# cxjyxxme/deep-online-video-stabilization

Measured on AMD Instinct MI355X. Metric: stabilized frames/sec (720p, before_ch=31), higher is better.
Workload: dtype f32 (bf16x3 split MFMA, f32 accumulate); 1 GPU; BASELINE.json configs[1]: v2_93 net, 1280x720, 1 stream(s)/GPU, batch=1 per stream, 13-ch stack from a 32-deep ring (lags 1,2,4,8,16,32; --before-ch 31 ignored as in the reference), ResNet-v2-50 regressor + 4x4 multi-grid warp + feedback; one independent stream set per GPU (replicas only); height=720, width=1280, streams_per_gpu=1, refine=1, operand_mode=4, launches_per_frame=64, hip_graph=True

## Files before the change

deep-online-video-stabilization_amd/csrc/conv.h:

```cpp
#pragma once
#include "common.h"

struct ConvArgs {
    const float* x;
    const float* w;
    float* y;
    const float* bias;
    const float* in_scale;
    const float* in_shift;
    const float* residual;
    const float* out_scale;
    const float* out_shift;
    const float* out_floor;
    float* partial;
    int N, H, W, Cin, Ho, Wo, Cout, KH, KW, stride, pad;
    int up;
    int res_H, res_W, res_stride;
    int relu_out;
    int x_ld, res_ld;
    int M, K;
    int splitk, steps_per_split;
    int cin_real;
    unsigned div_hw_mul, div_hw_shift, div_w_mul, div_w_shift;
    int rowrun;
    int in_scale_expected;
    int xcd_swizzle;
};

size_t conv_plan(ConvArgs& a);
struct Prof;
int conv_launch(const ConvArgs& a, hipStream_t st, Prof* prof = nullptr, int bf16_operands = 0, const float* w_img = nullptr,
                bool lowk_ring = false);

enum ConvFamily {
    CONV_IGEMM,
    CONV_RING,
    CONV_RING_KG,
    CONV_RING_PRO,
    CONV_PACKED,
    CONV_PACKED_KG2,
    CONV_ASTAT,
    CONV_PATCH
};
struct ConvRoute {
    int family;
    int tile, bk, nbuf;
    int mode;
    int operand;
    int kg, pro;
    int reduce;
    int prof_kind;
    int astat_bm;
    int patch_cfg;
};
ConvRoute conv_route(const ConvArgs& a, int operand_mode, bool has_image, bool bound, bool lowk_ring = false );
const char* conv_prof_kind_name(int kind);
size_t conv_weight_image_floats(int Cout, int K);
int launch_weight_split_image(const float* w, int Cout, int K, float* img, hipStream_t st);
struct WeightImageTable { long w_off[64], img_off[64], tprefix[65]; int Cout[64], K[64]; int n; };
void weight_image_table_add(WeightImageTable& t, long w_off, long img_off, int Cout, int K);
int launch_weight_split_images(const float* w_base, float* img_base, const WeightImageTable& t, hipStream_t st);
int conv_reduce_launches(const ConvArgs& a, int operand_mode = 0);

struct ConvPair { int m_tower, x_tower_floats ; long dx, dy, dres, dscale; };
bool conv_pair_supported(const ConvArgs& a);
int conv_launch_pair(const ConvArgs& a, const ConvPair& pr, hipStream_t st, Prof* prof = nullptr,
                     const float* w_img = nullptr );

bool conv_b2b_supported(const ConvArgs& c2, const ConvArgs& c3);
int conv_b2b_launch(const ConvArgs& c2, const ConvArgs& c3, hipStream_t st, Prof* prof = nullptr);

static inline void sn_fastdiv_make(unsigned d, unsigned& mul, unsigned& shift) {
    unsigned l = 0;
    while ((1ull << l) < d) ++l;
    mul = (unsigned)((((1ull << l) - d) << 32) / d + 1);
    shift = l;
}
#ifdef __HIPCC__
__device__ __forceinline__ int sn_fastdiv(int n, unsigned mul, unsigned shift) {
    return (int)((__umulhi(mul, (unsigned)n) + (unsigned)n) >> shift);
}
#endif
```

deep-online-video-stabilization_amd/csrc/conv.hip:

```cpp
#include "conv.h"
#include "prof.h"
#include <climits>
#include <cstdio>
#include <cstdlib>
#include <algorithm>
#include <string>
#include <vector>

#include "conv_kernel.h"
#include "conv_ring_kernel.h"
#include "conv_astat_kernel.h"
#include "conv_patch_kernel.h"
#include "conv_b2b_kernel.h"

template <int PAIR>
__device__ __forceinline__ void conv_splitk_reduce_body(const ConvArgs& p, const ConvPair& pr) {
    const size_t q = (size_t)blockIdx.x * 256 + threadIdx.x;
    const int c4n = p.Cout / 4;
    if (q >= (size_t)p.M * c4n) return;
    const int m = (int)(q / c4n);
    const int n = (int)(q - (size_t)m * c4n) * 4;
    const bool t1 = PAIR && m >= pr.m_tower;
    const size_t slab = (size_t)p.M * p.Cout;
    const float* src = p.partial + (size_t)m * p.Cout + n;
    float4 s = *reinterpret_cast<const float4*>(src);
    for (int z = 1; z < p.splitk; ++z) {
        const float4 t = *reinterpret_cast<const float4*>(src + z * slab);
        s.x += t.x; s.y += t.y; s.z += t.z; s.w += t.w;
    }
    if (p.bias != nullptr) {
        const float4 b = *reinterpret_cast<const float4*>(p.bias + n);
        s.x += b.x; s.y += b.y; s.z += b.z; s.w += b.w;
    }
    if (p.residual != nullptr) {
        size_t ri;
        if (p.res_stride == 1 && p.res_H == p.Ho && p.res_W == p.Wo) {
            ri = (size_t)m * p.res_ld + n;
        } else {
            const int img = sn_fastdiv(m, p.div_hw_mul, p.div_hw_shift);
            const int rr = m - img * (p.Ho * p.Wo);
            const int oy = sn_fastdiv(rr, p.div_w_mul, p.div_w_shift), ox = rr - oy * p.Wo;
            ri = (((size_t)img * p.res_H + oy * p.res_stride) * p.res_W + ox * p.res_stride) * p.res_ld + n;
        }
        const float4 t = *reinterpret_cast<const float4*>(p.residual + (t1 ? pr.dres : 0) + ri);
        s.x += t.x; s.y += t.y; s.z += t.z; s.w += t.w;
    }
    if (p.out_scale != nullptr) {
        const float4 a = *reinterpret_cast<const float4*>(p.out_scale + n), b = *reinterpret_cast<const float4*>(p.out_shift + n);
        s.x = __builtin_fmaf(s.x, a.x, b.x); s.y = __builtin_fmaf(s.y, a.y, b.y);
        s.z = __builtin_fmaf(s.z, a.z, b.z); s.w = __builtin_fmaf(s.w, a.w, b.w);
    }
    if (p.out_scale != nullptr && p.out_floor != nullptr) {
        const float4 f = *reinterpret_cast<const float4*>(p.out_floor + n);
        s.x = fmaxf(s.x, f.x); s.y = fmaxf(s.y, f.y); s.z = fmaxf(s.z, f.z); s.w = fmaxf(s.w, f.w);
    } else if (p.relu_out) {
        s.x = fmaxf(s.x, 0.f); s.y = fmaxf(s.y, 0.f); s.z = fmaxf(s.z, 0.f); s.w = fmaxf(s.w, 0.f);
    }
    *reinterpret_cast<float4*>(p.y + (t1 ? pr.dy : 0) + (size_t)m * p.Cout + n) = s;
}
__global__ __launch_bounds__(256) void conv_splitk_reduce_kernel(const ConvArgs p) {
    conv_splitk_reduce_body<0>(p, ConvPair{});
}
__global__ __launch_bounds__(256) void conv_splitk_reduce_pair_kernel(const ConvArgs p, const ConvPair pr) {
    conv_splitk_reduce_body<1>(p, pr);
}

enum TileId { T128x128 = 0, T128x64 = 1, T64x64 = 2 };

static void tile_dims(int t, int& bm, int& bn) {
    bm = (t == T64x64) ? 64 : 128;
    bn = (t == T128x128) ? 128 : 64;
}

static int env_int(const char* name, int dflt) {
    const char* v = getenv(name);
    return v ? atoi(v) : dflt;
}

struct ConvSwitches {
    int tile = env_int("STABNET_CONV_TILE", -1), splitk = env_int("STABNET_CONV_SPLITK", -1);
    int bk16 = env_int("STABNET_CONV_BK16", 0);
    int nbuf = env_int("STABNET_CONV_NBUF", 0);
    int tuning_table = env_int("STABNET_CONV_TUNING_TABLE", 1);
    int split_below = env_int("STABNET_CONV_SPLIT_BELOW", 400), split_target = env_int("STABNET_CONV_SPLIT_TARGET", 448);
    int xcd = env_int("STABNET_CONV_XCD", 1);
    int ring = env_int("STABNET_CONV_RING", 1), ring_wgs_per_cu = env_int("STABNET_CONV_RING_WGS_PER_CU", 3);
    int lowk_igemm = env_int("STABNET_CONV_LOWK_IGEMM", 1);
    int ring_pro = env_int("STABNET_CONV_RING_PRO", 1);
    int kgroups = env_int("STABNET_CONV_KGROUPS", 1), kgroups_pro = env_int("STABNET_CONV_KGROUPS_PRO", 1);
    int packed_kg2 = env_int("STABNET_CONV_PACKED_KG2", 1), packed_kg3 = env_int("STABNET_CONV_PACKED_KG3", 1);
    int packed_pro = env_int("STABNET_CONV_PACKED_PRO", 1);
    int packed_wgs_per_cu = env_int("STABNET_CONV_PACKED_WGS_PER_CU", 2);
    int astat = env_int("STABNET_CONV_ASTAT", 1), astat_min_m = env_int("STABNET_CONV_ASTAT_MIN_M", 0);
    int astat_min_cout = env_int("STABNET_CONV_ASTAT_MIN_COUT", 256);
    int patch = env_int("STABNET_CONV_PATCH", 1), patch_min_m = env_int("STABNET_CONV_PATCH_MIN_M", 0);
    int patch_cfg = env_int("STABNET_CONV_PATCH_CFG", 0);
    int b2b = env_int("STABNET_CONV_B2B", 1), b2b_wgs_per_cu = env_int("STABNET_CONV_B2B_WGS_PER_CU", 2);
};
static const ConvSwitches& sw() {
    static const ConvSwitches s;
    return s;
}

static int g_force_tile = -2, g_force_split = -1;
static int force_tile() { return g_force_tile == -2 ? sw().tile : g_force_tile; }
static int force_split() { return g_force_tile == -2 ? sw().splitk : g_force_split; }

static int conv_bk(const ConvArgs& a) { return (a.rowrun || (a.Cin % 32 == 0 && !sw().bk16)) ? 32 : 16; }
static int conv_total_steps(const ConvArgs& a) {
    if (a.rowrun) return a.KH * cdiv(a.KW * a.Cin, 32);
    return a.KH * a.KW * (a.Cin / conv_bk(a));
}

struct TuneEntry { int M, Cout, K, KH, ring, splitk; };
#include "conv_tuning_table.h"
#include "conv_tuning_table_packed.h"
static int g_tuning_profile = 0;
static std::vector<TuneEntry> g_tuning_runtime;

static int tuning_lookup(int M, int Cout, int K, int KH, int ring) {
    for (const TuneEntry& e : g_tuning_runtime)
        if (e.M == M && e.Cout == Cout && e.K == K && e.KH == KH && e.ring == ring) return e.splitk;
    if (sw().tuning_table && g_tuning_profile == 1)
        for (const TuneEntry& e : g_tuning_packed)
            if (e.M == M && e.Cout == Cout && e.K == K && e.KH == KH && e.ring == ring) return e.splitk;
    if (sw().tuning_table)
        for (const TuneEntry& e : g_tuning_builtin)
            if (e.M == M && e.Cout == Cout && e.K == K && e.KH == KH && e.ring == ring) return e.splitk;
    return 0;
}

static int pick_tile(const ConvArgs& a, int& splitk) {
    if (force_tile() >= 0) {
        const int steps0 = conv_total_steps(a);
        splitk = force_split() > 0 ? std::min(force_split(), steps0) : 1;
        return force_tile();
    }
    const int total_steps = conv_total_steps(a);
    const long blocks = (long)cdiv(a.M, 64) * cdiv(a.Cout, 64);
    const bool ring_path = a.rowrun || (a.in_scale_expected == 0 && a.up == 1 && a.Cin % 32 == 0);
    int s = tuning_lookup(a.M, a.Cout, a.K, a.KH, ring_path ? 1 : 0);
    const int thr = sw().split_below, target = sw().split_target;
    if (s > 0) {
        s = std::min(s, std::max(1, total_steps / 2));
    } else if (blocks < thr && a.Cout % 4 == 0) {
        s = (int)((target + blocks / 2) / blocks);
        s = std::min(s, std::max(1, total_steps / 8));
        s = std::min(s, 32);
    } else {
        s = 1;
    }
    splitk = std::max(1, s);
    return T64x64;
}

size_t conv_plan(ConvArgs& a) {
    a.xcd_swizzle = sw().xcd;
    a.M = a.N * a.Ho * a.Wo;
    a.K = a.rowrun ? a.KH * 32 * cdiv(a.KW * a.Cin, 32) : a.KH * a.KW * a.Cin;
    if (a.x_ld == 0) a.x_ld = a.Cin;
    if (a.res_ld == 0) a.res_ld = a.Cout;
    sn_fastdiv_make((unsigned)(a.Ho * a.Wo), a.div_hw_mul, a.div_hw_shift);
    sn_fastdiv_make((unsigned)a.Wo, a.div_w_mul, a.div_w_shift);
    int splitk = 1;
    (void)pick_tile(a, splitk);
    const int total_steps = conv_total_steps(a);
    a.steps_per_split = cdiv(total_steps, splitk);
    a.splitk = cdiv(total_steps, a.steps_per_split);
    return a.splitk > 1 ? (size_t)a.splitk * a.M * a.Cout * sizeof(float) : 0;
}

static void igemm_variant(const ConvArgs& a, int bm, int bn, int bk, int mode, int operand, int& nbuf_out, int& bf16_out) {
    const int nbuf = sw().nbuf;
    bf16_out = (bm == 64 && bn == 64 && bk == 32) ? operand : 0;
    const bool one_stage = nbuf == 1 || (nbuf == 0 && mode == 0 && bm == 64 && bn == 64 && a.M >= 32768);
    nbuf_out = (bf16_out != 1 && one_stage) ? 1 : 2;
}

static bool ring_eligible(const ConvArgs& a, int tile, bool has_prologue, bool lowk_ring = false) {
    if (a.rowrun) return true;
    if (!lowk_ring && sw().lowk_igemm && a.KH == 1 && a.KW == 1 && a.Cin == 64 && a.x_ld == a.Cin && a.out_floor == nullptr) return false;
    return sw().ring && tile == T64x64 && !has_prologue && a.up == 1 && a.Cin % 32 == 0 && !sw().bk16;
}

static bool ring_pro_vectors_ok(const ConvArgs& a) {
    if (a.in_scale == nullptr || a.in_shift == nullptr) return true;
    const long d = (long)(a.in_shift - a.in_scale);
    return d >= 0 && d < (1L << 30);
}
static bool ring_pro_geometry(const ConvArgs& a, int operand, bool has_prologue) {
    return sw().ring_pro && sw().ring && operand != 1 && !sw().bk16 && has_prologue && a.KH == 1 && a.KW == 1 && a.stride == 1 && a.pad == 0 &&
           a.up == 1 && a.Cin % 32 == 0 && !a.rowrun && a.x_ld == a.Cin;
}
static bool ring_pro_eligible(const ConvArgs& a, int operand) {
    return ring_pro_geometry(a, operand, a.in_scale != nullptr) && a.out_scale == nullptr && a.out_floor == nullptr && ring_pro_vectors_ok(a);
}

static int conv_kgroups(const ConvArgs& a, int operand, bool ring, bool has_prologue) {
    if (!sw().kgroups || a.splitk < 2 || operand == 1) return 1;
    if (a.steps_per_split * a.splitk != conv_total_steps(a)) return 1;
    if (ring && a.splitk == 3 && !a.rowrun) return 3;
    if (sw().kgroups_pro && !ring && a.splitk == 2 && ring_pro_geometry(a, operand, has_prologue) && ring_pro_vectors_ok(a)) return 2;
    return 1;
}

struct PatchForm { int ph, pw, wr, ns; };
static const PatchForm g_patch_forms[] = {{8, 8, 1, 3}, {8, 8, 2, 3}};
constexpr int SN_PATCH_FORMS = 2;
constexpr size_t SN_PATCH_LDS_MAX = 160 * 1024;
static int patch_cfg(const ConvArgs& a) {
    auto fits = [&](int cfg) { return sn_patch_lds_bytes(g_patch_forms[cfg - 1].ph, g_patch_forms[cfg - 1].pw, a.Cin) <= SN_PATCH_LDS_MAX; };
    const int forced = sw().patch_cfg;
    if (forced >= 1 && forced <= SN_PATCH_FORMS) return fits(forced) ? forced : 0;
    const int cfg = a.Cout <= 64 ? 1 : 2;
    return fits(cfg) ? cfg : 0;
}

static int route_prof_kind(const ConvRoute& r) {
    switch (r.family) {
        case CONV_IGEMM:
            return PK_KERNEL_CONV_BASE + r.mode * 6 + r.tile * 2 + (r.bk == 32 ? 1 : 0) + (r.nbuf == 1 ? 18 : 0) + 36 * r.operand;
        case CONV_PACKED: return PK_KERNEL_CONV_PACKED + (r.pro ? 3 : r.mode);
        case CONV_PACKED_KG2: return PK_KERNEL_CONV_PACKED + (r.pro ? 6 : 4 + r.mode);
        case CONV_ASTAT: return PK_KERNEL_CONV_ASTAT;
        case CONV_PATCH: return PK_KERNEL_CONV_PATCH + r.patch_cfg - 1;
        default: break;
    }
    const int split = r.operand >= 2 ? PK_KERNEL_CONV_SPLIT + 8 * (r.operand - 2) : 0;
    if (r.family == CONV_RING) return split ? split + r.mode : PK_KERNEL_CONV_RING + r.mode + (r.operand ? 3 : 0);
    if (r.family == CONV_RING_PRO) return split ? split + 5 : PK_KERNEL_CONV_KG + 2;
    if (r.kg == 2) return split ? split + 6 : PK_KERNEL_CONV_KG + 3;
    return split ? split + 3 + r.mode : PK_KERNEL_CONV_KG + r.mode;
}

ConvRoute conv_route(const ConvArgs& a, int operand_mode, bool has_image, bool bound, bool lowk_ring) {
    const ConvSwitches& s = sw();
    const bool image = operand_mode == 4 && has_image;
    const int op = operand_mode == 4 ? 0 : operand_mode;
    int splitk_unused = 1;
    const int t = pick_tile(a, splitk_unused);
    const bool t64 = t == T64x64, bk32 = conv_bk(a) == 32;
    const bool has_pro = bound ? a.in_scale != nullptr : a.in_scale_expected != 0;
    const bool ring = ring_eligible(a, t, has_pro, lowk_ring && image);
    const bool slabs = !bound || a.splitk == 1 || a.partial != nullptr;
    int kg = t64 ? conv_kgroups(a, op, ring, has_pro) : 1;
    if (image && s.packed_kg3 && ring && kg == 3 && a.K % 32 == 0 && slabs) kg = 1;
    const bool pro = kg == 1 && !ring && t64 && bk32 && (bound ? ring_pro_eligible(a, op) : ring_pro_geometry(a, op, has_pro));
    const bool packed_pro = image && s.packed_pro && !ring && t64 && bk32 && ring_pro_geometry(a, op, has_pro) &&
                            (!bound || a.out_floor == nullptr)  && ring_pro_vectors_ok(a) && slabs;
    if (packed_pro) kg = 1;
    const bool packed = (image && ring && kg == 1 && a.K % 32 == 0) || packed_pro;
    const bool packed_kg2 = packed && s.packed_kg2 && a.splitk == 2 && !a.rowrun && a.steps_per_split * 2 == conv_total_steps(a);
    if (packed_kg2) kg = 2;
    const int astat_min_m = s.astat_min_m > 0 ? s.astat_min_m : ((long)a.Cout * a.K >= 128 * 1024 ? 2048 : 8192);
    const bool astat = packed && !packed_pro && !packed_kg2 && kg == 1 && a.splitk == 1 && s.astat && !lowk_ring && !a.rowrun &&
                       a.KH == 1 && a.KW == 1 && a.stride == 1 && a.pad == 0 && a.up == 1 && a.K <= 256 && a.Cout >= s.astat_min_cout &&
                       a.M >= astat_min_m;
    const int patch_form = patch_cfg(a);
    const bool patch = packed && !packed_pro && ((kg == 1 && a.splitk == 1) || packed_kg2) && s.patch && !lowk_ring && !a.rowrun &&
                       a.KH == 3 && a.KW == 3 && a.stride == 1 && a.pad == 1 && a.up == 1 && a.Cin % 32 == 0 && patch_form != 0 &&
                       a.M >= (s.patch_min_m > 0 ? s.patch_min_m : 12288);

    ConvRoute r{};
    r.tile = t;
    r.bk = bk32 ? 32 : 16;
    r.mode = (a.up > 1 || a.rowrun) ? 2 : (a.pad == 0 ? 0 : 1);
    r.operand = op;
    r.kg = kg;
    r.reduce = (a.splitk > 1 && kg == 1) ? 1 : 0;
    if (astat) {
        r.family = CONV_ASTAT;
        r.operand = 4;
        r.astat_bm = 32;
    } else if (patch) {
        r.family = CONV_PATCH;
        r.operand = 4;
        r.patch_cfg = patch_form;
    } else if (packed) {
        r.family = packed_kg2 ? CONV_PACKED_KG2 : CONV_PACKED;
        r.operand = 4;
        r.pro = packed_pro ? 1 : 0;
    } else if (pro) {
        r.family = CONV_RING_PRO;
        r.pro = 1;
    } else if (kg > 1) {
        r.family = CONV_RING_KG;
        r.pro = kg == 2 ? 1 : 0;
    } else if (ring) {
        r.family = CONV_RING;
    } else {
        int bm, bn;
        tile_dims(t, bm, bn);
        r.family = CONV_IGEMM;
        igemm_variant(a, bm, bn, r.bk, r.mode, op, r.nbuf, r.operand);
    }
    r.prof_kind = route_prof_kind(r);
    return r;
}

int conv_reduce_launches(const ConvArgs& a, int operand_mode) {
    return a.splitk < 2 ? 0 : conv_route(a, operand_mode, operand_mode == 4, false).reduce;
}

const char* conv_prof_kind_name(int kind) {
    static const std::vector<std::string> names = [] {
        std::vector<std::string> v(PK_KERNEL_CONV_BASE + 144);
        char buf[96];
        auto ring = [&](int family, int mode, int operand, int kg, int pro) {
            ConvRoute r{};
            r.family = family; r.mode = mode; r.operand = operand; r.kg = kg; r.pro = pro;
            snprintf(buf, sizeof(buf), "conv_ring_f32_kernel<%d, %d, %d, %d>", mode, operand, kg, pro);
            v[route_prof_kind(r)] = buf;
        };
        for (int operand = 0; operand < 4; ++operand) {
            for (int mode = 0; mode < 3; ++mode) ring(CONV_RING, mode, operand, 1, 0);
            if (operand == 1) continue;
            ring(CONV_RING_KG, 0, operand, 3, 0); ring(CONV_RING_KG, 1, operand, 3, 0);
            ring(CONV_RING_PRO, 0, operand, 1, 1); ring(CONV_RING_KG, 0, operand, 2, 1);
        }
        for (int mode = 0; mode < 3; ++mode) ring(CONV_PACKED, mode, 4, 1, 0);
        ring(CONV_PACKED, 0, 4, 1, 1);
        ring(CONV_PACKED_KG2, 0, 4, 2, 0); ring(CONV_PACKED_KG2, 1, 4, 2, 0); ring(CONV_PACKED_KG2, 0, 4, 2, 1);
        {
            ConvRoute r{};
            r.family = CONV_ASTAT; r.astat_bm = 32;
            snprintf(buf, sizeof(buf), "conv_astat_f32_kernel<%d>", r.astat_bm);
            v[route_prof_kind(r)] = buf;
        }
        for (int cfg = 1; cfg <= SN_PATCH_FORMS; ++cfg) {
            ConvRoute r{};
            r.family = CONV_PATCH; r.patch_cfg = cfg;
            const PatchForm& f = g_patch_forms[cfg - 1];
            snprintf(buf, sizeof(buf), "conv_patch_f32_kernel<%d, %d, %d, %d>", f.ph, f.pw, f.wr, f.ns);
            v[route_prof_kind(r)] = buf;
        }
        for (int i = 0; i < 144; ++i) {
            ConvRoute r{};
            r.family = CONV_IGEMM;
            r.operand = i / 36; r.nbuf = 2 - i / 18 % 2; r.mode = i / 6 % 3; r.tile = i / 2 % 3; r.bk = (i & 1) ? 32 : 16;
            int bm, bn;
            tile_dims(r.tile, bm, bn);
            snprintf(buf, sizeof(buf), "conv_igemm_f32_kernel<%d, %d, %d, %d, %d, %d, %d, %d>", bm, bn, r.bk, bm / 2, bn / 2, r.mode, r.nbuf, r.operand);
            v[route_prof_kind(r)] = buf;
        }
        for (int i = 0; i < 4; ++i) {
            snprintf(buf, sizeof(buf), "conv_igemm_f32_pair_kernel<64, 64, %d, 32, 32, %d>", (i & 1) ? 32 : 16, i / 2);
            v[PK_KERNEL_CONV_PAIR + i] = buf;
        }
        v[PK_KERNEL_CONV_B2B] = "conv_b2b_f32_kernel<2>";
        v[PK_KERNEL_CONV_B2B + 1] = "conv_b2b_f32_kernel<4>";
        return v;
    }();
    return (kind >= 0 && kind < (int)names.size() && !names[kind].empty()) ? names[kind].c_str() : nullptr;
}

template <int BM, int BN, int BK, int WM, int WN, int MODE, int NBUF, int BF16 = 0>
static int launch_one_nb(const ConvArgs& a, hipStream_t st) {
    constexpr size_t lds_op = NBUF * (size_t)(BM + BN) * (BK + 4) * sizeof(float);
    constexpr size_t lds_epi = 4 * (size_t)SN_EPI_WAVE_BYTES;
    constexpr size_t lds = lds_op > lds_epi ? lds_op : lds_epi;
    static bool configured = false;
    auto kern = conv_igemm_f32_kernel<BM, BN, BK, WM, WN, MODE, NBUF, BF16>;
    if (!configured) {
        if (lds > 64 * 1024) {
            hipError_t e = hipFuncSetAttribute(reinterpret_cast<const void*>(kern),
                                               hipFuncAttributeMaxDynamicSharedMemorySize, (int)lds);
            if (e != hipSuccess) {
                stabnet_set_error("conv: hipFuncSetAttribute(%zu B LDS) failed: %s", lds, hipGetErrorString(e));
                return STABNET_ERR_LAUNCH;
            }
        }
        configured = true;
    }
    dim3 grid(cdiv(a.M, BM), cdiv(a.Cout, BN), a.splitk);
    kern<<<grid, 256, lds, st>>>(a);
    SN_LAUNCH_CHECK("conv_igemm_f32_kernel");
    return STABNET_OK;
}

template <int BM, int BN, int BK, int WM, int WN, int MODE>
static int launch_one_t(const ConvRoute& r, const ConvArgs& a, hipStream_t st) {
    if constexpr (BM == 64 && BN == 64 && BK == 32) {
        if (r.operand == 1) return launch_one_nb<BM, BN, BK, WM, WN, MODE, 2, 1>(a, st);
        else if (r.operand == 2) return r.nbuf == 1 ? launch_one_nb<BM, BN, BK, WM, WN, MODE, 1, 2>(a, st) : launch_one_nb<BM, BN, BK, WM, WN, MODE, 2, 2>(a, st);
        else if (r.operand == 3) return r.nbuf == 1 ? launch_one_nb<BM, BN, BK, WM, WN, MODE, 1, 3>(a, st) : launch_one_nb<BM, BN, BK, WM, WN, MODE, 2, 3>(a, st);
    }
    return r.nbuf == 1 ? launch_one_nb<BM, BN, BK, WM, WN, MODE, 1>(a, st) : launch_one_nb<BM, BN, BK, WM, WN, MODE, 2>(a, st);
}

template <int BM, int BN, int BK, int WM, int WN>
static int launch_one(const ConvRoute& r, const ConvArgs& a, hipStream_t st) {
    if (r.mode == 2) return launch_one_t<BM, BN, BK, WM, WN, 2>(r, a, st);
    if (r.mode == 0) return launch_one_t<BM, BN, BK, WM, WN, 0>(r, a, st);
    return launch_one_t<BM, BN, BK, WM, WN, 1>(r, a, st);
}

static int launch_igemm(const ConvRoute& r, const ConvArgs& a, hipStream_t st) {
    if (r.bk == 32) {
        if (r.tile == T128x128) return launch_one<128, 128, 32, 64, 64>(r, a, st);
        if (r.tile == T128x64) return launch_one<128, 64, 32, 64, 32>(r, a, st);
        return launch_one<64, 64, 32, 32, 32>(r, a, st);
    }
    if (r.tile == T128x128) return launch_one<128, 128, 16, 64, 64>(r, a, st);
    if (r.tile == T128x64) return launch_one<128, 64, 16, 64, 32>(r, a, st);
    return launch_one<64, 64, 16, 32, 32>(r, a, st);
}

static int device_cus(int& cus) {
    static int cached = 0;
    if (cached == 0) {
        int dev = 0, n = 0;
        if (hipGetDevice(&dev) != hipSuccess || hipDeviceGetAttribute(&n, hipDeviceAttributeMultiprocessorCount, dev) != hipSuccess || n <= 0) {
            stabnet_set_error("conv: cannot read the CU count");
            return STABNET_ERR_LAUNCH;
        }
        cached = n;
    }
    cus = cached;
// ... 11 lines not shown
    if constexpr (B != 1) {
        if (key == 11) { conv_ring_f32_kernel<0, B, 1, 1><<<grid, 256, 0, st>>>(a); return true; }
        if (key == 21) { conv_ring_f32_kernel<0, B, 2, 1><<<grid, 512, 0, st>>>(a); return true; }
    }
    if constexpr (B == 0 || B == 2 || B == 3) {
        if (key == 30) { conv_ring_f32_kernel<0, B, 3><<<grid, 768, 0, st>>>(a); return true; }
        if (key == 130) { conv_ring_f32_kernel<1, B, 3><<<grid, 768, 0, st>>>(a); return true; }
    }
    if constexpr (B == 4) {
        if (key == 20) { conv_ring_f32_kernel<0, B, 2, 0><<<grid, 512, 0, st>>>(a); return true; }
        if (key == 120) { conv_ring_f32_kernel<1, B, 2, 0><<<grid, 512, 0, st>>>(a); return true; }
    }
    return false;
}

static int launch_ring_route(const ConvRoute& r, const ConvArgs& a, hipStream_t st) {
    int cus = 0;
    if (const int rc = device_cus(cus)) return rc;
    const int per_cu = r.kg > 1 ? 1 : (r.operand == 4 ? sw().packed_wgs_per_cu : sw().ring_wgs_per_cu);
    const long ntiles = (long)cdiv(a.M, 64) * cdiv(a.Cout, 64) * (r.kg > 1 ? 1 : a.splitk);
    const int grid = (int)std::min<long>(ntiles, (long)per_cu * usable_cus(cus));
    bool ok = false;
    switch (r.operand) {
        case 0: ok = launch_ring_operand<0>(r, a, grid, st); break;
        case 1: ok = launch_ring_operand<1>(r, a, grid, st); break;
        case 2: ok = launch_ring_operand<2>(r, a, grid, st); break;
        case 3: ok = launch_ring_operand<3>(r, a, grid, st); break;
        case 4: ok = launch_ring_operand<4>(r, a, grid, st); break;
        default: break;
    }
    SN_REQUIRE(ok, "conv: no conv_ring_f32_kernel<%d, %d, %d, %d>", r.mode, r.operand, r.kg, r.pro);
    SN_LAUNCH_CHECK("conv_ring_f32_kernel");
    return STABNET_OK;
}

static int launch_astat(const ConvRoute& r, const ConvArgs& a, hipStream_t st) {
    int cus = 0;
    if (const int rc = device_cus(cus)) return rc;
    const int bm = r.astat_bm;
    SN_REQUIRE(bm == 32 && a.K % 32 == 0 && (size_t)bm * a.K * 6 <= (size_t)SN_ASTAT_A_BYTES && a.splitk == 1,
               "conv: the A-stationary kernel takes BM %d x K %d without a K split only if the planes fit %d bytes", bm, a.K, SN_ASTAT_A_BYTES);
    const int mtiles = cdiv(a.M, bm), nblk = 2 * cdiv(a.Cout, 64);
    int groups = (int)std::min<long>(cdiv(nblk, 4), std::max<long>(1, 2L * usable_cus(cus) / mtiles));
    groups = cdiv(nblk, 4 * cdiv(cdiv(nblk, groups), 4));
    const dim3 grid(mtiles, groups);
    conv_astat_f32_kernel<32><<<grid, 256, 0, st>>>(a);
    SN_LAUNCH_CHECK("conv_astat_f32_kernel");
    return STABNET_OK;
}

template <int PH, int PW, int WR, int NS>
static int launch_patch_one(const ConvArgs& a, int cus, hipStream_t st) {
    const size_t lds = sn_patch_lds_bytes(PH, PW, a.Cin);
    auto kern = conv_patch_f32_kernel<PH, PW, WR, NS>;
    static size_t configured = 64 * 1024;
    if (lds > configured) {
        hipError_t e = hipFuncSetAttribute(reinterpret_cast<const void*>(kern), hipFuncAttributeMaxDynamicSharedMemorySize, (int)SN_PATCH_LDS_MAX);
        if (e != hipSuccess) {
            stabnet_set_error("conv: hipFuncSetAttribute(%zu B LDS) failed: %s", SN_PATCH_LDS_MAX, hipGetErrorString(e));
            return STABNET_ERR_LAUNCH;
        }
        configured = SN_PATCH_LDS_MAX;
    }
    constexpr int cs = 4 / ((PH / 4) * (PW / 8) / WR);
    const int mtiles = a.N * cdiv(a.Ho, PH) * cdiv(a.Wo, PW), nblk = 2 * cdiv(a.Cout, 64);
    const long slots = (long)std::min<size_t>(WR >= 4 ? 1 : 2, SN_PATCH_LDS_MAX / lds) * usable_cus(cus);
    int groups = (int)std::min<long>(cdiv(nblk, cs), std::max<long>(1, slots / mtiles));
    groups = cdiv(nblk, cs * cdiv(cdiv(nblk, groups), cs));
    const dim3 grid(mtiles, groups);
    kern<<<grid, 256, lds, st>>>(a);
    SN_LAUNCH_CHECK("conv_patch_f32_kernel");
    return STABNET_OK;
}
static int launch_patch(const ConvRoute& r, const ConvArgs& a, hipStream_t st) {
    int cus = 0;
    if (const int rc = device_cus(cus)) return rc;
    SN_REQUIRE(a.KH == 3 && a.KW == 3 && a.stride == 1 && a.pad == 1 && a.up == 1 && a.Cin % 32 == 0 &&
                   (a.splitk == 1 || (a.splitk == 2 && a.steps_per_split * 2 == conv_total_steps(a))) && a.Ho == a.H && a.Wo == a.W && r.patch_cfg >= 1 &&
                   r.patch_cfg <= SN_PATCH_FORMS &&
                   sn_patch_lds_bytes(g_patch_forms[r.patch_cfg - 1].ph, g_patch_forms[r.patch_cfg - 1].pw, a.Cin) <= SN_PATCH_LDS_MAX,
               "conv: the patch-stationary kernel takes 3x3 / pad 1 / stride 1 over Cin %d (a multiple of 32) without a K split or with two equal K halves only if the planes fit %zu bytes",
               a.Cin, SN_PATCH_LDS_MAX);
    return r.patch_cfg == 1 ? launch_patch_one<8, 8, 1, 3>(a, cus, st) : launch_patch_one<8, 8, 2, 3>(a, cus, st);
}

size_t conv_weight_image_floats(int Cout, int K) { return (size_t)cdiv(Cout, 64) * (size_t)(K / 32) * 3072; }

__device__ __forceinline__ unsigned weight_split_head(float& x0, float& x1) {
    const float top = __builtin_bit_cast(float, 0x7F7F0000u), fmax = __builtin_bit_cast(float, 0x7F7FFFFFu);
    const float h0 = (fabsf(x0) > top && fabsf(x0) <= fmax) ? copysignf(top, x0) : x0;
    const float h1 = (fabsf(x1) > top && fabsf(x1) <= fmax) ? copysignf(top, x1) : x1;
    const unsigned p = sn_pack_bf16(h0, h1);
    x0 = sn_sub_f32(x0, __builtin_bit_cast(float, p << 16));
    x1 = sn_sub_f32(x1, __builtin_bit_cast(float, p & 0xffff0000u));
    return p;
}
__device__ __forceinline__ SnSplit3 weight_split3(const f32x4 x) {
    float a = x.x, b = x.y, c = x.z, d = x.w;
    typedef unsigned u32x2 __attribute__((ext_vector_type(2)));
    u32x2 h, m, l;
    h.x = weight_split_head(a, b); h.y = weight_split_head(c, d);
    m.x = sn_split_level(a, b); m.y = sn_split_level(c, d);
    l.x = sn_pack_bf16(a, b); l.y = sn_pack_bf16(c, d);
    SnSplit3 s;
    s.h = __builtin_bit_cast(sn_bf16x4, h); s.m = __builtin_bit_cast(sn_bf16x4, m); s.l = __builtin_bit_cast(sn_bf16x4, l);
    return s;
}

__device__ __forceinline__ void weight_split_image_thread(const float* __restrict__ w, int Cout, int K, uint4* __restrict__ img, long i) {
    const int steps = K / 32;
    const int lane = (int)(i & 63), j = (int)((i >> 6) & 1), wn = (int)((i >> 7) & 1);
    const long ts = i >> 8;
    const int ks = (int)(ts % steps), nt = (int)(ts / steps);
    const int n = nt * 64 + wn * 32 + (lane & 31), g = lane >> 5;
    f32x4 lo = {0.f, 0.f, 0.f, 0.f}, hi = lo;
    if (n < Cout) {
        const float* r = w + (size_t)n * K + ks * 32 + 16 * j + 4 * g;
        lo = *reinterpret_cast<const f32x4*>(r);
        hi = *reinterpret_cast<const f32x4*>(r + 8);
    }
    const SnSplit3 a = weight_split3(lo), b = weight_split3(hi);
    uint4* out = img + ts * 768 + (size_t)(wn * 6 + j) * 64 + lane;
    out[0] = __builtin_bit_cast(uint4, SN_CAT8(a.h, b.h));
    out[2 * 64] = __builtin_bit_cast(uint4, SN_CAT8(a.m, b.m));
    out[4 * 64] = __builtin_bit_cast(uint4, SN_CAT8(a.l, b.l));
}

__global__ __launch_bounds__(256) void weight_split_image_kernel(const float* __restrict__ w, int Cout, int K, uint4* __restrict__ img) {
    const long i = (long)blockIdx.x * 256 + threadIdx.x;
    if (i >= (long)((Cout + 63) / 64) * (K / 32) * 256) return;
    weight_split_image_thread(w, Cout, K, img, i);
}

__global__ __launch_bounds__(256) void weight_split_images_kernel(const float* __restrict__ w_base, float* __restrict__ img_base, const WeightImageTable t) {
    const long i = (long)blockIdx.x * 256 + threadIdx.x;
    if (i >= t.tprefix[t.n]) return;
    int e = 0;
    while (i >= t.tprefix[e + 1]) ++e;
    weight_split_image_thread(w_base + t.w_off[e], t.Cout[e], t.K[e], reinterpret_cast<uint4*>(img_base + t.img_off[e]), i - t.tprefix[e]);
}

void weight_image_table_add(WeightImageTable& t, long w_off, long img_off, int Cout, int K) {
    if (t.n == 0) t.tprefix[0] = 0;
    t.w_off[t.n] = w_off; t.img_off[t.n] = img_off; t.Cout[t.n] = Cout; t.K[t.n] = K;
    t.tprefix[t.n + 1] = t.tprefix[t.n] + (long)cdiv(Cout, 64) * (K / 32) * 256;
    ++t.n;
}

int launch_weight_split_images(const float* w_base, float* img_base, const WeightImageTable& t, hipStream_t st) {
    if (t.n == 0) return STABNET_OK;
    SN_REQUIRE(w_base && img_base && t.n <= 64, "weight images: bad table");
    weight_split_images_kernel<<<(unsigned)(t.tprefix[t.n] >> 8), 256, 0, st>>>(w_base, img_base, t);
    SN_LAUNCH_CHECK("weight_split_images_kernel");
    return STABNET_OK;
}

int launch_weight_split_image(const float* w, int Cout, int K, float* img, hipStream_t st) {
    SN_REQUIRE(w && img && Cout > 0 && K > 0 && K % 32 == 0, "weight image: K=%d must be a multiple of 32", K);
    const long total = (long)cdiv(Cout, 64) * (K / 32) * 256;
    weight_split_image_kernel<<<cdiv(total, 256), 256, 0, st>>>(w, Cout, K, reinterpret_cast<uint4*>(img));
    SN_LAUNCH_CHECK("weight_split_image_kernel");
    return STABNET_OK;
}

int conv_launch(const ConvArgs& a, hipStream_t st, Prof* prof, int bf16_operands, const float* w_img, bool lowk_ring) {
    SN_REQUIRE(a.rowrun || a.Cin % 16 == 0, "conv: Cin=%d must be a multiple of 16 (pad the channels)", a.Cin);
    SN_REQUIRE(!a.rowrun || (a.in_scale == nullptr && a.up == 1 && a.KH <= 8 && cdiv(a.KW * a.Cin, 32) <= 4),
               "conv: row-run operand needs no prologue, KH <= 8 and KW*Cin <= 128");
    SN_REQUIRE(a.Cout % 4 == 0, "conv: Cout=%d must be a multiple of 4", a.Cout);
    SN_REQUIRE(a.splitk >= 1 && a.steps_per_split >= 1 && a.div_hw_mul != 0, "conv: conv_plan() not called");
    SN_REQUIRE(a.splitk == 1 || a.partial != nullptr, "conv: split-K needs a workspace");
    const ConvRoute r = conv_route(a, bf16_operands, w_img != nullptr, true, lowk_ring);
    SN_REQUIRE(r.family != CONV_IGEMM || a.x_ld == a.Cin, "conv: a strided input (x_ld %d != Cin %d) needs the ring kernel", a.x_ld, a.Cin);
    const bool rec = prof != nullptr && prof->begin(st);
    int rc;
    switch (r.family) {
        case CONV_IGEMM: rc = launch_igemm(r, a, st); break;
        case CONV_PACKED:
        case CONV_PACKED_KG2: {
            ConvArgs b = a;
            b.w = w_img;
            rc = launch_ring_route(r, b, st);
            break;
        }
        case CONV_ASTAT: {
            ConvArgs b = a;
            b.w = w_img;
            rc = launch_astat(r, b, st);
            break;
        }
        case CONV_PATCH: {
            ConvArgs b = a;
            b.w = w_img;
            rc = launch_patch(r, b, st);
            break;
        }
        default: rc = launch_ring_route(r, a, st); break;
    }
    if (rec) prof->end(st, r.prof_kind, 2.0 * a.M * (double)(a.KH * a.KW * (a.cin_real ? a.cin_real : a.Cin)) * a.Cout,
                       4.0 * ((double)a.N * a.H * a.W * a.Cin + (double)a.K * a.Cout + (double)a.M * a.Cout * (r.reduce ? a.splitk : 1) +
                              ((a.residual != nullptr && !r.reduce) ? (double)a.M * a.Cout : 0.0)),
                       a.M, a.Cout, a.K, a.splitk);
    if (rc) return rc;
    if (r.reduce) {
        const size_t q = (size_t)a.M * (a.Cout / 4);
        const bool rec2 = prof != nullptr && prof->begin(st);
        conv_splitk_reduce_kernel<<<cdiv((long)q, 256), 256, 0, st>>>(a);
        if (rec2) prof->end(st, PK_KERNEL_SPLITK_REDUCE, 0.0, 4.0 * (double)a.M * a.Cout * (a.splitk + 1 + (a.residual != nullptr ? 1 : 0)));
        SN_LAUNCH_CHECK("conv_splitk_reduce_kernel");
    }
    return STABNET_OK;
}

bool conv_pair_supported(const ConvArgs& a) {
    int splitk_unused = 1;
    const int t = pick_tile(a, splitk_unused);
    const bool pro = a.in_scale != nullptr || a.in_scale_expected;
    return t == T64x64 && !ring_eligible(a, t, pro) && a.up == 1 && !a.rowrun && (a.x_ld == 0 || a.x_ld == a.Cin);
}

template <int BK, int MODE>
static int launch_pair_one(const ConvArgs& a, const ConvPair& pr, hipStream_t st) {
    constexpr size_t lds = 2 * (size_t)(64 + 64) * (BK + 4) * sizeof(float);
    static_assert(lds >= 4 * (size_t)SN_EPI_WAVE_BYTES && lds <= 64 * 1024, "LDS of the 64x64 tile");
    dim3 grid(cdiv(a.M, 64), cdiv(a.Cout, 64), a.splitk);
    conv_igemm_f32_pair_kernel<64, 64, BK, 32, 32, MODE><<<grid, 256, lds, st>>>(a, pr);
    SN_LAUNCH_CHECK("conv_igemm_f32_pair_kernel");
    return STABNET_OK;
}

int conv_launch_pair(const ConvArgs& a, const ConvPair& pr, hipStream_t st, Prof* prof, const float* w_img) {
    SN_REQUIRE(a.Cin % 16 == 0 && a.Cout % 4 == 0, "conv pair: Cin %% 16 and Cout %% 4 must be 0");
    SN_REQUIRE(a.splitk >= 1 && a.steps_per_split >= 1 && a.div_hw_mul != 0, "conv pair: conv_plan() not called");
    SN_REQUIRE(a.splitk == 1 || a.partial != nullptr, "conv pair: split-K needs a workspace");
    SN_REQUIRE(conv_pair_supported(a), "conv pair: the plan of this shape is not the 64x64 register-staged launch");
    SN_REQUIRE(pr.m_tower > 0 && pr.m_tower % 64 == 0 && a.M == 2 * pr.m_tower, "conv pair: tower rows %d must be a multiple of 64 (M %d)",
               pr.m_tower, a.M);
    const bool bk32 = conv_bk(a) == 32;
    const int mode = a.pad == 0 ? 0 : 1;
    const bool pro = bk32 && ring_pro_eligible(a, 0) && pr.dx == pr.dscale - (long)pr.m_tower * a.Cin && pr.dy == pr.dscale - (long)pr.m_tower * a.Cout &&
                     (a.residual == nullptr || pr.dres == pr.dscale - (long)(a.N / 2) * a.res_H * a.res_W * a.res_ld);
    const bool packed = pro && w_img != nullptr && a.K % 32 == 0 && a.splitk == 1;
    ConvRoute r{};
    r.family = packed ? CONV_PACKED : CONV_RING_PRO;
    r.operand = packed ? 4 : 0;
    r.kg = r.pro = 1;
    const bool rec = prof != nullptr && prof->begin(st);
    int rc;
    if (pro) {
        ConvArgs b = a;
        b.out_floor = reinterpret_cast<const float*>((size_t)pr.dscale);
        if (packed) b.w = w_img;
        rc = launch_ring_route(r, b, st);
    } else if (bk32) {
        rc = mode == 0 ? launch_pair_one<32, 0>(a, pr, st) : launch_pair_one<32, 1>(a, pr, st);
    } else {
        rc = mode == 0 ? launch_pair_one<16, 0>(a, pr, st) : launch_pair_one<16, 1>(a, pr, st);
    }
    if (rec) prof->end(st, pro ? route_prof_kind(r) : PK_KERNEL_CONV_PAIR + mode * 2 + (bk32 ? 1 : 0), 2.0 * a.M * (double)(a.KH * a.KW * (a.cin_real ? a.cin_real : a.Cin)) * a.Cout,
                       4.0 * ((double)a.N * a.H * a.W * a.Cin + (double)a.K * a.Cout + (double)a.M * a.Cout * a.splitk),
                       a.M, a.Cout, a.K, a.splitk);
    if (rc) return rc;
    if (a.splitk > 1) {
        const size_t q = (size_t)a.M * (a.Cout / 4);
        const bool rec2 = prof != nullptr && prof->begin(st);
        conv_splitk_reduce_pair_kernel<<<cdiv((long)q, 256), 256, 0, st>>>(a, pr);
        if (rec2) prof->end(st, PK_KERNEL_SPLITK_REDUCE, 0.0, 4.0 * (double)a.M * a.Cout * (a.splitk + 1));
        SN_LAUNCH_CHECK("conv_splitk_reduce_pair_kernel");
    }
    return STABNET_OK;
}

bool conv_b2b_supported(const ConvArgs& c2, const ConvArgs& c3) {
    const bool g2 = c2.KH == 3 && c2.KW == 3 && c2.pad == 1 && c2.up == 1 && !c2.rowrun && (c2.stride == 1 || c2.stride == 2) &&
                    c2.Cin == c2.Cout && (c2.Cout == 64 || c2.Cout == 128) && c2.in_scale_expected == 0 && c2.in_scale == nullptr;
    const bool g3 = c3.KH == 1 && c3.KW == 1 && c3.pad == 0 && c3.stride == 1 && c3.up == 1 && !c3.rowrun && c3.Cin == c2.Cout &&
                    (c3.x_ld == 0 || c3.x_ld == c3.Cin) && c3.Cout % c2.Cout == 0 && c3.N == c2.N && c3.H == c2.Ho && c3.W == c2.Wo &&
// ... 226 lines not shown
```

deep-online-video-stabilization_amd/csrc/prof.h:

```cpp
#pragma once
#include <vector>
#include "common.h"

enum {
    PK_KERNEL_PAD = 1, PK_KERNEL_POOL = 2, PK_KERNEL_GAP = 3, PK_KERNEL_FC = 4, PK_KERNEL_MESH = 5,
    PK_KERNEL_WARP = 6, PK_KERNEL_ASSEMBLE = 7, PK_KERNEL_PUSH = 8, PK_KERNEL_SPLITK_REDUCE = 9, PK_KERNEL_WGRAD = 10, PK_KERNEL_HEAD = 20,
    PK_KERNEL_MJPEG_TRANSFORM = 30, PK_KERNEL_MJPEG_ENTROPY = 31, PK_KERNEL_MJPEG_LAYOUT = 32, PK_KERNEL_MJPEG_GATHER = 33 ,
    PK_KERNEL_INGEST_GREY_ROWS = 34, PK_KERNEL_INGEST_GREY_COLS = 35, PK_KERNEL_INGEST_COLOUR = 36 ,
    PK_KERNEL_MAP_SHRINK = 37, PK_KERNEL_REMAP_SRC = 38, PK_KERNEL_REMAP_SRC4 = 39 ,
    PK_KERNEL_REMAP_WIN = 60, PK_KERNEL_REMAP_WIN4 = 61 ,
    PK_KERNEL_REMAP_WIN_DEV = 62, PK_KERNEL_REMAP_WIN4_DEV = 63 ,
    PK_KERNEL_REMAP_I420 = 59 ,
    PK_KERNEL_TF_GET_IMG = 64,
    PK_KERNEL_TVL1_STEP = 57, PK_KERNEL_TVL1_FUSED = 58 ,
    PK_KERNEL_TVL1_DOWN = 65, PK_KERNEL_TVL1_GRAD = 66, PK_KERNEL_TVL1_WARP = 67, PK_KERNEL_TVL1_UP = 68, PK_KERNEL_TVL1_MAP = 69 ,
    PK_KERNEL_KLT_DETECT = 26, PK_KERNEL_KLT_TRACK = 27, PK_KERNEL_KLT_FINISH = 28 ,
    PK_KERNEL_HOMFIT = 29 ,
    PK_KERNEL_WGRAD_SAME = 11 ,
    PK_KERNEL_CONV_PAIR = 80 , PK_KERNEL_CONV_KG = 84 , PK_KERNEL_CONV_RING = 90 ,
    PK_KERNEL_CONV_PACKED = 70 ,
    PK_KERNEL_CONV_ASTAT = 77 ,
    PK_KERNEL_CONV_PATCH = 24 ,
    PK_KERNEL_CONV_B2B = 96 ,
    PK_KERNEL_CONV_SPLIT = 40 ,
    PK_KERNEL_CONV_BASE = 100
};

struct Prof {
    std::vector<hipEvent_t> ev;
    std::vector<int> kind;
    std::vector<double> flops, bytes;
    std::vector<int> shape;
    int cap = 0, n = 0;
    bool begin(hipStream_t st) {
        if (n >= cap) return false;
        (void)hipEventRecord(ev[2 * n], st);
        return true;
    }
    void end(hipStream_t st, int k, double f, double b, int sm = 0, int sn = 0, int sk = 0, int ss = 0) {
        (void)hipEventRecord(ev[2 * n + 1], st);
        kind[n] = k; flops[n] = f; bytes[n] = b;
        shape[4 * n] = sm; shape[4 * n + 1] = sn; shape[4 * n + 2] = sk; shape[4 * n + 3] = ss;
        ++n;
    }
};
```

Before: 725.0 frames/s.

## Add K-streaming 1x1 conv kernel with prologue fusion and deep prefetch

Adds a new conv family for 1x1 stride-1 convolutions with a fused BN+ReLU prologue. It streams the K dimension through double-buffered LDS, with register prefetch of activations up to four steps ahead and weights two steps ahead, and a small BM tile. The bf16x3 split happens at publish time. The kernel is routed ahead of the packed path whenever the packed-prologue route would apply and M is large enough. The aim is to hide global-load latency for bandwidth-bound 1x1 convs. It adds another code path and per-wave tiling choices that may be less efficient than the existing packed kernel for some shapes.

```diff
diff --git a/deep-online-video-stabilization_amd/csrc/conv.h b/deep-online-video-stabilization_amd/csrc/conv.h
--- a/deep-online-video-stabilization_amd/csrc/conv.h
+++ b/deep-online-video-stabilization_amd/csrc/conv.h
@@ -40,7 +40,8 @@
     CONV_PACKED,
     CONV_PACKED_KG2,
     CONV_ASTAT,
-    CONV_PATCH
+    CONV_PATCH,
+    CONV_KSTREAM
 };
 struct ConvRoute {
     int family;
@@ -52,6 +53,7 @@
     int prof_kind;
     int astat_bm;
     int patch_cfg;
+    int kstream_cfg;
 };
 ConvRoute conv_route(const ConvArgs& a, int operand_mode, bool has_image, bool bound, bool lowk_ring = false );
 const char* conv_prof_kind_name(int kind);
diff --git a/deep-online-video-stabilization_amd/csrc/conv.hip b/deep-online-video-stabilization_amd/csrc/conv.hip
--- a/deep-online-video-stabilization_amd/csrc/conv.hip
+++ b/deep-online-video-stabilization_amd/csrc/conv.hip
@@ -11,6 +11,7 @@
 #include "conv_ring_kernel.h"
 #include "conv_astat_kernel.h"
 #include "conv_patch_kernel.h"
+#include "conv_kstream_kernel.h"
 #include "conv_b2b_kernel.h"
 
 template <int PAIR>
@@ -95,6 +96,8 @@
     int astat_min_cout = env_int("STABNET_CONV_ASTAT_MIN_COUT", 256);
     int patch = env_int("STABNET_CONV_PATCH", 1), patch_min_m = env_int("STABNET_CONV_PATCH_MIN_M", 0);
     int patch_cfg = env_int("STABNET_CONV_PATCH_CFG", 0);
+    int kstream = env_int("STABNET_CONV_KSTREAM", 1), kstream_min_m = env_int("STABNET_CONV_KSTREAM_MIN_M", 0);
+    int kstream_cfg = env_int("STABNET_CONV_KSTREAM_CFG", 0);
     int b2b = env_int("STABNET_CONV_B2B", 1), b2b_wgs_per_cu = env_int("STABNET_CONV_B2B_WGS_PER_CU", 2);
 };
 static const ConvSwitches& sw() {
@@ -216,6 +219,16 @@
     return fits(cfg) ? cfg : 0;
 }
 
+struct KstreamForm { int bm, wr; };
+static const KstreamForm g_kstream_forms[] = {{64, 1}, {64, 2}, {32, 1}};
+constexpr int SN_KSTREAM_FORMS = 3;
+static int kstream_cfg(const ConvArgs& a) {
+    const int forced = sw().kstream_cfg;
+    if (forced >= 1 && forced <= SN_KSTREAM_FORMS) return forced;
+    if (a.Cout <= 64) return 1;
+    return a.M >= 8192 ? 2 : 3;
+}
+
 static int route_prof_kind(const ConvRoute& r) {
     switch (r.family) {
         case CONV_IGEMM:
@@ -224,6 +237,7 @@
         case CONV_PACKED_KG2: return PK_KERNEL_CONV_PACKED + (r.pro ? 6 : 4 + r.mode);
         case CONV_ASTAT: return PK_KERNEL_CONV_ASTAT;
         case CONV_PATCH: return PK_KERNEL_CONV_PATCH + r.patch_cfg - 1;
+        case CONV_KSTREAM: return PK_KERNEL_CONV_KSTREAM + r.kstream_cfg - 1;
         default: break;
     }
     const int split = r.operand >= 2 ? PK_KERNEL_CONV_SPLIT + 8 * (r.operand - 2) : 0;
@@ -260,6 +274,10 @@
     const bool patch = packed && !packed_pro && ((kg == 1 && a.splitk == 1) || packed_kg2) && s.patch && !lowk_ring && !a.rowrun &&
                        a.KH == 3 && a.KW == 3 && a.stride == 1 && a.pad == 1 && a.up == 1 && a.Cin % 32 == 0 && patch_form != 0 &&
                        a.M >= (s.patch_min_m > 0 ? s.patch_min_m : 12288);
+    const int kstream_floor = s.kstream_min_m > 0 ? s.kstream_min_m : (a.K >= 1024 ? 3072 : 12288);
+    const bool kstream = packed_pro && ((kg == 1 && a.splitk == 1) || packed_kg2) && s.kstream && !lowk_ring && a.M >= kstream_floor &&
+                         (size_t)a.M * a.K < (1ull << 30) && conv_weight_image_floats(a.Cout, a.K) < (1ull << 30)  &&
+                         (!bound || (((size_t)a.in_scale | (size_t)a.in_shift | (size_t)a.x) & 15) == 0);
 
     ConvRoute r{};
     r.tile = t;
@@ -276,6 +294,11 @@
         r.family = CONV_PATCH;
         r.operand = 4;
         r.patch_cfg = patch_form;
+    } else if (kstream) {
+        r.family = CONV_KSTREAM;
+        r.operand = 4;
+        r.pro = 1;
+        r.kstream_cfg = kstream_cfg(a);
     } else if (packed) {
         r.family = packed_kg2 ? CONV_PACKED_KG2 : CONV_PACKED;
         r.operand = 4;
@@ -334,6 +357,12 @@
             snprintf(buf, sizeof(buf), "conv_patch_f32_kernel<%d, %d, %d, %d>", f.ph, f.pw, f.wr, f.ns);
             v[route_prof_kind(r)] = buf;
         }
+        for (int cfg = 1; cfg <= SN_KSTREAM_FORMS; ++cfg) {
+            ConvRoute r{};
+            r.family = CONV_KSTREAM; r.kstream_cfg = cfg;
+            snprintf(buf, sizeof(buf), "conv_kstream_f32_kernel<%d, %d>", g_kstream_forms[cfg - 1].bm, g_kstream_forms[cfg - 1].wr);
+            v[route_prof_kind(r)] = buf;
+        }
         for (int i = 0; i < 144; ++i) {
             ConvRoute r{};
             r.family = CONV_IGEMM;
@@ -511,6 +540,25 @@
                "conv: the patch-stationary kernel takes 3x3 / pad 1 / stride 1 over Cin %d (a multiple of 32) without a K split or with two equal K halves only if the planes fit %zu bytes",
                a.Cin, SN_PATCH_LDS_MAX);
     return r.patch_cfg == 1 ? launch_patch_one<8, 8, 1, 3>(a, cus, st) : launch_patch_one<8, 8, 2, 3>(a, cus, st);
+}
+
+template <int BM, int WR>
+static int launch_kstream_one(const ConvArgs& a, hipStream_t st) {
+    constexpr int bn = 32 * 4 / (BM / 32 / WR);
+    const dim3 grid(cdiv(a.M, BM), cdiv(a.Cout, bn));
+    conv_kstream_f32_kernel<BM, WR><<<grid, 256, 0, st>>>(a);
+    SN_LAUNCH_CHECK("conv_kstream_f32_kernel");
+    return STABNET_OK;
+}
+static int launch_kstream(const ConvRoute& r, const ConvArgs& a, hipStream_t st) {
+    SN_REQUIRE(a.KH == 1 && a.KW == 1 && a.stride == 1 && a.pad == 0 && a.up == 1 && !a.rowrun && a.Cin % 32 == 0 && a.x_ld == a.Cin &&
+                   a.in_scale != nullptr && a.in_shift != nullptr && a.out_floor == nullptr &&
+                   (a.splitk == 1 || (a.splitk == 2 && a.steps_per_split * 2 == conv_total_steps(a))) && r.kstream_cfg >= 1 &&
+                   r.kstream_cfg <= SN_KSTREAM_FORMS && (size_t)a.M * a.K < (1ull << 30) && conv_weight_image_floats(a.Cout, a.K) < (1ull << 30),
+               "conv: the K-streaming kernel takes 1x1 / stride 1 over dense Cin %d (a multiple of 32) with a prologue, without a K split or with two equal K halves, below 4 GiB of input and of weight image",
+               a.Cin);
+    if (r.kstream_cfg == 1) return launch_kstream_one<64, 1>(a, st);
+    return r.kstream_cfg == 2 ? launch_kstream_one<64, 2>(a, st) : launch_kstream_one<32, 1>(a, st);
 }
 
 size_t conv_weight_image_floats(int Cout, int K) { return (size_t)cdiv(Cout, 64) * (size_t)(K / 32) * 3072; }
@@ -622,6 +670,12 @@
             ConvArgs b = a;
             b.w = w_img;
             rc = launch_patch(r, b, st);
+            break;
+        }
+        case CONV_KSTREAM: {
+            ConvArgs b = a;
+            b.w = w_img;
+            rc = launch_kstream(r, b, st);
             break;
         }
         default: rc = launch_ring_route(r, a, st); break;
diff --git a/deep-online-video-stabilization_amd/csrc/conv_kstream_kernel.h b/deep-online-video-stabilization_amd/csrc/conv_kstream_kernel.h
--- /dev/null
+++ b/deep-online-video-stabilization_amd/csrc/conv_kstream_kernel.h
@@ -0,0 +1,171 @@
+#pragma once
+#include "conv_kernel.h"
+
+#ifndef KSTREAM_ABLATE
+#define KSTREAM_ABLATE 0
+#endif
+#ifdef KSTREAM_STAMP
+__device__ unsigned long long* g_kstream_stamps;
+#define KSTREAM_STAMP_AT(i)                                                                                               \
+    do {                                                                                                                  \
+        if (threadIdx.x == 0) g_kstream_stamps[(size_t)(blockIdx.x + gridDim.x * blockIdx.y) * 4 + (i)] = __builtin_amdgcn_s_memtime(); \
+    } while (0)
+#else
+#define KSTREAM_STAMP_AT(i)
+#endif
+
+template <int BM , int WR >
+__global__ __launch_bounds__(256, 2) void conv_kstream_f32_kernel(const ConvArgs p) {
+    static_assert((BM == 32 || BM == 64) && (WR == 1 || WR == 2) && (BM / 32) % WR == 0, "one or two 32-row blocks, one or two per wave");
+    constexpr int RB = BM / 32, RU = RB / WR, NW = 4 / RU;
+    constexpr int STAGE = RB * 2 * 3072;
+    typedef unsigned u32x2 __attribute__((ext_vector_type(2)));
+    __shared__ __attribute__((aligned(16))) unsigned char lds[2 * STAGE + 4 * SN_EPI_WAVE_BYTES];
+
+    const int tid = threadIdx.x, lane = tid & 63, wave = __builtin_amdgcn_readfirstlane(tid >> 6);
+    const int steps = p.K >> 5;
+    const ConvTile tile = conv_tile_of_block(p);
+    const int m0 = tile.mt * BM;
+    const int ru = wave % RU, b = tile.nt * NW + wave / RU;
+    const bool live = b * 32 < p.Cout;
+    const int bimg = min(b, 2 * ((p.Cout + 63) >> 6) - 1);
+    KSTREAM_STAMP_AT(0);
+
+    const int r = tid >> 3, sub = tid & 7;
+    const unsigned ent = (unsigned)((sub >> 2) * 3072 + (r + 32 * (sub & 1)) * 16 + 8 * ((sub >> 1) & 1));
+    unsigned src[RB];
+#pragma unroll
+    for (int rb = 0; rb < RB; ++rb) src[rb] = ((unsigned)min(m0 + rb * 32 + r, p.M - 1) * (unsigned)p.x_ld + (unsigned)(sub * 4)) * 4u;
+    const unsigned scoff = (unsigned)(sub * 16);
+    const char* const xb = reinterpret_cast<const char*>(p.x);
+    const char* const scb = reinterpret_cast<const char*>(p.in_scale);
+    const char* const shb = reinterpret_cast<const char*>(p.in_shift);
+    struct AStage { f32x4 v[RB], sc, sh; };
+    auto aload = [&](AStage& s, int ks) {
+        const size_t k = (size_t)(128 * min(ks, steps - 1));
+        if (!(KSTREAM_ABLATE & 1)) {
+#pragma unroll
+            for (int rb = 0; rb < RB; ++rb) s.v[rb] = *reinterpret_cast<const f32x4*>(xb + k + src[rb]);
+            s.sc = *reinterpret_cast<const f32x4*>(scb + k + scoff);
+            s.sh = *reinterpret_cast<const f32x4*>(shb + k + scoff);
+        } else {
+#pragma unroll
+            for (int rb = 0; rb < RB; ++rb) s.v[rb] = f32x4{(float)k, (float)r, (float)sub, 1.f};
+            s.sc = f32x4{1.f, -1.f, 1.f, -1.f};
+            s.sh = f32x4{0.f, 0.f, 0.f, 0.f};
+        }
+    };
+    auto publish = [&](const AStage& s, unsigned buf ) {
+#pragma unroll
+        for (int rb = 0; rb < RB; ++rb) {
+            float a = fmaxf(__builtin_fmaf(s.v[rb].x, s.sc.x, s.sh.x), 0.f), b2 = fmaxf(__builtin_fmaf(s.v[rb].y, s.sc.y, s.sh.y), 0.f);
+            float c = fmaxf(__builtin_fmaf(s.v[rb].z, s.sc.z, s.sh.z), 0.f), d = fmaxf(__builtin_fmaf(s.v[rb].w, s.sc.w, s.sh.w), 0.f);
+            u32x2 h, m, l;
+            h.x = sn_split_level(a, b2); h.y = sn_split_level(c, d);
+            m.x = sn_split_level(a, b2); m.y = sn_split_level(c, d);
+            l.x = sn_pack_bf16(a, b2); l.y = sn_pack_bf16(c, d);
+            unsigned char* dst = lds + (buf + (unsigned)(rb * 6144) + ent);
+            *reinterpret_cast<u32x2*>(dst) = h;
+            *reinterpret_cast<u32x2*>(dst + 1024) = m;
+            *reinterpret_cast<u32x2*>(dst + 2048) = l;
+        }
+    };
+
+    const char* const bp = reinterpret_cast<const char*>(p.w) + ((size_t)(bimg >> 1) * steps * 12 + (bimg & 1) * 6) * 1024;
+    const unsigned boff = (unsigned)(lane * 16);
+    auto bload = [&](f32x4 (&dst)[6], int ks) {
+        if ((KSTREAM_ABLATE & 2) && ks >= 2) return;
+        const char* lp = bp + (size_t)min(ks, steps - 1) * 12288;
+#pragma unroll
+        for (int i = 0; i < 6; ++i) dst[i] = *reinterpret_cast<const f32x4*>(lp + i * 1024 + boff);
+        __builtin_amdgcn_sched_barrier(0);
+    };
+
+    f32x16 acc[WR][1], first_half[WR];
+    const int half = p.splitk == 2 ? steps >> 1 : steps;
+#pragma unroll
+    for (int i = 0; i < WR; ++i)
+#pragma unroll
+        for (int e = 0; e < 16; ++e) { acc[i][0][e] = 0.f; first_half[i][e] = 0.f; }
+    const unsigned char* const afrag = lds + (unsigned)(ru * WR * 6144 + lane * 16);
+    auto multiply = [&](const f32x4 (&B)[6], unsigned buf) {
+#pragma unroll
+        for (int j = 0; j < 2; ++j) {
+            SnPlanes A[WR];
+#pragma unroll
+            for (int i = 0; i < WR; ++i) {
+                const unsigned char* ap = afrag + (buf + (unsigned)((i * 2 + j) * 3072));
+                A[i].h = *reinterpret_cast<const sn_u32x4*>(ap);
+                A[i].m = *reinterpret_cast<const sn_u32x4*>(ap + 1024);
+                A[i].l = *reinterpret_cast<const sn_u32x4*>(ap + 2048);
+            }
+            const sn_bf16x8 bh = __builtin_bit_cast(sn_bf16x8, B[j]), bm = __builtin_bit_cast(sn_bf16x8, B[2 + j]), bl = __builtin_bit_cast(sn_bf16x8, B[4 + j]);
+#define SN_KSTREAM_MFMA(ap_, b_)                                                                                                    \
+    _Pragma("unroll") for (int i = 0; i < WR; ++i)                                                                                  \
+        acc[i][0] = __builtin_amdgcn_mfma_f32_32x32x16_bf16(__builtin_bit_cast(sn_bf16x8, A[i].ap_), b_, acc[i][0], 0, 0, 0)
+            SN_KSTREAM_MFMA(l, bh);
+            SN_KSTREAM_MFMA(h, bl);
+            SN_KSTREAM_MFMA(m, bm);
+            SN_KSTREAM_MFMA(m, bh);
+            SN_KSTREAM_MFMA(h, bm);
+            SN_KSTREAM_MFMA(h, bh);
+#undef SN_KSTREAM_MFMA
+        }
+    };
+    auto step = [&](int s, AStage& S, f32x4 (&Bl)[6], const f32x4 (&Bm)[6], bool fetch , bool pub ) {
+        const unsigned buf = (unsigned)((s & 1) * STAGE);
+        __syncthreads();
+        if (fetch) bload(Bl, s + 2);
+        multiply(Bm, buf);
+        if (pub) publish(S, buf ^ (unsigned)STAGE);
+        if (fetch) aload(S, s + 4);
+        __builtin_amdgcn_sched_barrier(0);
+        if (s + 1 == half && half != steps) {
+            __builtin_amdgcn_sched_barrier(0);
+#pragma unroll
+            for (int i = 0; i < WR; ++i) {
+                first_half[i] = acc[i][0];
+#pragma unroll
+                for (int e2 = 0; e2 < 16; ++e2) acc[i][0][e2] = 0.f;
+            }
+        }
+    };
+
+    AStage S0, S1, S2;
+    f32x4 B0[6], B1[6], B2[6];
+    aload(S0, 0);
+    aload(S1, 1);
+    aload(S2, 2);
+    bload(B0, 0);
+    bload(B1, 1);
+    publish(S0, 0u);
+    KSTREAM_STAMP_AT(1);
+    aload(S0, 3);
+    int s = 0;
+    for (; s + 3 <= steps; s += 3) {
+        step(s, S1, B2, B0, true, true);
+        step(s + 1, S2, B0, B1, true, true);
+        step(s + 2, S0, B1, B2, true, true);
+    }
+    if (s + 2 == steps) {
+        step(s, S1, B2, B0, false, true);
+        step(s + 1, S2, B0, B1, false, false);
+    } else if (s + 1 == steps) {
+        step(s, S1, B2, B0, false, false);
+    }
+    KSTREAM_STAMP_AT(2);
+    if (live) {
+        if (half != steps) {
+#pragma unroll
+            for (int i = 0; i < WR; ++i)
+#pragma unroll
+                for (int e = 0; e < 16; ++e) acc[i][0][e] = first_half[i][e] + acc[i][0][e];
+        }
+        const unsigned scratch = (unsigned)(size_t)(__attribute__((address_space(3))) void*)lds + (unsigned)(2 * STAGE + wave * SN_EPI_WAVE_BYTES);
+        conv_epilogue<WR, 1, true>(acc, p, m0 + ru * WR * 32, b * 32, lane, 0, scratch);
+    }
+#ifdef KSTREAM_STAMP
+    __syncthreads();
+    KSTREAM_STAMP_AT(3);
+#endif
+}
diff --git a/deep-online-video-stabilization_amd/csrc/prof.h b/deep-online-video-stabilization_amd/csrc/prof.h
--- a/deep-online-video-stabilization_amd/csrc/prof.h
+++ b/deep-online-video-stabilization_amd/csrc/prof.h
@@ -21,6 +21,7 @@
     PK_KERNEL_CONV_PACKED = 70 ,
     PK_KERNEL_CONV_ASTAT = 77 ,
     PK_KERNEL_CONV_PATCH = 24 ,
+    PK_KERNEL_CONV_KSTREAM = 21 ,
     PK_KERNEL_CONV_B2B = 96 ,
     PK_KERNEL_CONV_SPLIT = 40 ,
     PK_KERNEL_CONV_BASE = 100
```

After: 725.7 frames/s, median of 3. About the same (+0.1%).
